# AleoNet/snarkVM

Hardware: NVIDIA H100
Metric: bls12_377_g1_msm_points_per_sec (higher is better)
Workload: dtype u32 limbs (Montgomery integer arithmetic, IMAD pipe)

## Files before the change

snarkvm_b200/csrc/msm.cu:

```cuda
#include "msm.cuh"

#include <atomic>
#include <condition_variable>
#include <memory>
#include <mutex>
#include <utility>
#include <vector>
#include <cstdio>
#include <cstdlib>
#include <cstring>
#include <cub/device/device_scan.cuh>

#define FF_CALL_MUL 1
#include "ec.cuh"
#include "cta_inverse.cuh"
#include "quad.cuh"
#define FIELD_TEST_ENTRY test_field_op_msm
#include "testops.cuh"

namespace b200 {

static std::atomic<uint64_t> g_launches{0};
uint64_t launch_count() { return g_launches.load(); }
void count_launch(int n) { g_launches.fetch_add((uint64_t)n); }
// ... 316 lines not shown
    acc.store(partial + (size_t)t * XYZZ_WORDS);
}

template <bool GATHER>
FF_DEV DensePoint load_level_input(const uint32_t* __restrict__ dense_bases, const uint32_t* __restrict__ sorted,
                                   const uint32_t* __restrict__ dense_in, uint32_t idx) {
    DensePoint d;
    if (GATHER) {
        uint32_t e = sorted[idx];
        d = load_dense(dense_bases + (size_t)(e & 0x7fffffffu) * BASE_WORDS);
        if ((e >> 31) && !d.inf) d.y = d.y.neg();
    } else {
        d = load_dense(dense_in + (size_t)idx * DENSE_WORDS);
    }
    return d;
}
template <bool GATHER>
FF_DEV const uint32_t* level_input_ptr(const uint32_t* __restrict__ dense_bases, const uint32_t* __restrict__ sorted,
                                       const uint32_t* __restrict__ dense_in, uint32_t idx) {
    if (GATHER) return dense_bases + (size_t)(sorted[idx] & 0x7fffffffu) * BASE_WORDS;
    return dense_in + (size_t)idx * DENSE_WORDS;
}
__global__ void k_densify_bases(const uint8_t* __restrict__ points, size_t stride, size_t n, uint32_t* __restrict__ out) {
    size_t i = (size_t)blockIdx.x * blockDim.x + threadIdx.x;
    if (i >= n) return;
    AffinePoint a = load_affine(points, stride, i);
    DensePoint d; d.x = a.x; d.y = a.y; d.inf = a.inf;
    store_dense(out + i * BASE_WORDS, d);
}
__global__ void __launch_bounds__(CTA_INV_THREADS) k_precompute_tables(const uint8_t* __restrict__ points, size_t stride, size_t n, int c, int nwin,
                                                            uint32_t* __restrict__ table) {
    __shared__ uint4 sh_inv[CTA_INV_SMEM_BYTES / 16];
    const size_t i = (size_t)blockIdx.x * blockDim.x + threadIdx.x;
    const bool live = i < n;
    AffinePoint a;
    a.x = Fq::zero(); a.y = Fq::zero(); a.inf = true;
    if (live) a = load_affine(points, stride, i);
    DensePoint d; d.x = a.x; d.y = a.y; d.inf = a.inf;
    if (live) store_dense(table + i * BASE_WORDS, d);
    XYZZ q = XYZZ::from_affine(a);
    for (int w = 1; w < nwin; w++) {
        for (int k = 0; k < c; k++) q.dbl();
        const bool inf = q.is_inf();
        Fq z = inf ? Fq::one() : q.ZZ * q.ZZZ;
        Fq iz = cta_shared_inverse_by(z, reinterpret_cast<uint32_t*>(sh_inv), w & 3);
        __syncthreads();
        if (inf) { d.x = Fq::zero(); d.y = Fq::zero(); d.inf = true; }
        else { d.x = q.X * (iz * q.ZZZ); d.y = q.Y * (iz * q.ZZ); d.inf = false; }
        if (live) store_dense(table + ((size_t)w * n + i) * BASE_WORDS, d);
    }
}

static constexpr int PAIR_THREADS = CTA_INV_THREADS;
enum PairKind { PAIR_COPY1 = 0, PAIR_COPY2 = 1, PAIR_INF = 2, PAIR_ADD = 3, PAIR_DBL = 4 };
FF_DEV int classify_pair(const DensePoint& P, const DensePoint& Q, bool has2, Fq& d) {
    if (!has2 || Q.inf) return PAIR_COPY1;
    if (P.inf) return PAIR_COPY2;
    if (P.x == Q.x) {
        if (P.y == Q.y && !P.y.is_zero()) { d = P.y.dbl(); return PAIR_DBL; }
        return PAIR_INF;
    }
    d = Q.x - P.x;
    return PAIR_ADD;
}

template <bool GATHER>
__global__ void __launch_bounds__(PAIR_THREADS, 4) k_pair_level(const uint32_t* __restrict__ dense_bases,
                                                        const uint32_t* __restrict__ sorted, const uint32_t* __restrict__ dense_in,
                                                        const uint32_t* __restrict__ off_in, const uint32_t* __restrict__ off_out,
                                                        uint32_t total_buckets, uint32_t T, uint32_t* __restrict__ prefix,
                                                        uint32_t* __restrict__ dense_out) {
    __shared__ uint4 sh_inv4[PAIR_THREADS * 3];
    uint32_t* sh_inv = reinterpret_cast<uint32_t*>(sh_inv4);
    const uint32_t total = off_out[total_buckets];
    const uint64_t o0_64 = (uint64_t)(blockIdx.x * blockDim.x + threadIdx.x) * T;
    const uint32_t o0 = o0_64 < total ? (uint32_t)o0_64 : total;
    const uint32_t o1 = (o0_64 + T < total) ? o0 + T : total;
    uint32_t lo = 0, hi = total_buckets;
    if (o0 < o1) while (hi - lo > 1) { uint32_t mid = (lo + hi) >> 1; if (off_out[mid] <= o0) lo = mid; else hi = mid; }
    uint32_t b = lo;

    Fq run = Fq::one();
    for (uint32_t o = o0; o < o1; o++) {
        while (o >= off_out[b + 1]) b++;
        const uint32_t i = o - off_out[b], base_in = off_in[b], cnt = off_in[b + 1] - base_in;
        const bool has2 = 2 * i + 1 < cnt;
        if (has2) {
            const uint32_t* pp = level_input_ptr<GATHER>(dense_bases, sorted, dense_in, base_in + 2 * i);
            const uint32_t* qp = level_input_ptr<GATHER>(dense_bases, sorted, dense_in, base_in + 2 * i + 1);
            Fq x1 = Fq::load_ldg(pp), x2 = Fq::load_ldg(qp);
            if (x1 == x2 || x1.is_zero() || x2.is_zero()) {
                DensePoint P = load_level_input<GATHER>(dense_bases, sorted, dense_in, base_in + 2 * i);
                DensePoint Q = load_level_input<GATHER>(dense_bases, sorted, dense_in, base_in + 2 * i + 1);
                Fq d;
                int kind = classify_pair(P, Q, true, d);
                if (kind >= PAIR_ADD) run = run * d;
            } else {
                run = run * (x2 - x1);
            }
        }
        run.store(prefix + (size_t)o * 12);
    }
    Fq inv = cta_shared_inverse(run, sh_inv);
    for (uint32_t o = o1; o-- > o0;) {
        while (o < off_out[b]) b--;
        const uint32_t i = o - off_out[b], base_in = off_in[b], cnt = off_in[b + 1] - base_in;
        const bool has2 = 2 * i + 1 < cnt;
        DensePoint P = load_level_input<GATHER>(dense_bases, sorted, dense_in, base_in + 2 * i);
        DensePoint Q = P;
        if (has2) Q = load_level_input<GATHER>(dense_bases, sorted, dense_in, base_in + 2 * i + 1);
        Fq d;
        int kind = classify_pair(P, Q, has2, d);
        DensePoint R;
        if (kind == PAIR_COPY1) R = P;
        else if (kind == PAIR_COPY2) R = Q;
        else if (kind == PAIR_INF) { R.inf = true; R.x = Fq::zero(); R.y = Fq::zero(); }
        else {
            Fq inv_d = (o == o0) ? inv : inv * Fq::load(prefix + (size_t)(o - 1) * 12);
            inv = inv * d;
            Fq lambda;
            if (kind == PAIR_ADD) lambda = (Q.y - P.y) * inv_d;
            else { Fq xx = P.x.sqr(); lambda = (xx.dbl() + xx) * inv_d; }
            Fq x3 = lambda.sqr() - P.x - Q.x;
            R.y = lambda * (P.x - x3) - P.y;
            R.x = x3;
            R.inf = false;
        }
        store_dense(dense_out + (size_t)o * DENSE_WORDS, R);
    }
}


FF_DEV uint32_t smem_addr_u32(const void* p) { return (uint32_t)__cvta_generic_to_shared(p); }
FF_DEV void cp_async16(uint32_t dst, const void* src) {
    asm volatile("cp.async.cg.shared.global [%0], [%1], 16;" ::"r"(dst), "l"(src) : "memory");
}
FF_DEV void cp_async_commit() { asm volatile("cp.async.commit_group;" ::: "memory"); }
FF_DEV void cp_async_wait_1() { asm volatile("cp.async.wait_group 1;" ::: "memory"); }
FF_DEV void cp_async_wait_0() { asm volatile("cp.async.wait_group 0;" ::: "memory"); }
FF_DEV void cp_async_wait_3() { asm volatile("cp.async.wait_group 3;" ::: "memory"); }

static constexpr int RING_CHUNKS = 12;
static constexpr int RING_STAGE_U4 = RING_CHUNKS * 32;
static constexpr int PAIR2_SMEM = PAIR_THREADS * 48 + 4 * 2 * RING_STAGE_U4 * 16;

FF_DEV Fq ring_fq(const uint4* slot) {
    Fq r;
#pragma unroll
    for (int i = 0; i < 3; i++) { uint4 t = slot[i * 32]; r.v[4 * i] = t.x; r.v[4 * i + 1] = t.y; r.v[4 * i + 2] = t.z; r.v[4 * i + 3] = t.w; }
    return r;
}

static constexpr uint32_t PAIR_NONE = 0xffffffffu;
template <bool GATHER>
__global__ void __launch_bounds__(256) k_pair_desc(const uint32_t* __restrict__ sorted, const uint32_t* __restrict__ off_in,
                                                   const uint32_t* __restrict__ off_out, uint32_t total_buckets, uint2* __restrict__ desc,
                                                   const uint32_t* __restrict__ in_base_ptr ) {
    const uint32_t o = blockIdx.x * blockDim.x + threadIdx.x;
    if (o >= __ldg(off_out + total_buckets)) return;
    uint32_t lo = 0, hi = total_buckets;
    while (hi - lo > 1) { uint32_t mid = (lo + hi) >> 1; if (__ldg(off_out + mid) <= o) lo = mid; else hi = mid; }
    const uint32_t i = o - __ldg(off_out + lo), base_in = __ldg(off_in + lo), cnt = __ldg(off_in + lo + 1) - base_in;
    const uint32_t idx = base_in + 2u * i;
    const bool has2 = 2u * i + 1u < cnt;
    uint2 d;
    if (GATHER) { d.x = __ldg(sorted + idx); d.y = has2 ? __ldg(sorted + idx + 1) : PAIR_NONE; }
    else { d.x = idx - (in_base_ptr ? __ldg(in_base_ptr) : 0u); d.y = has2 ? 0u : PAIR_NONE; }
    desc[o] = d;
}

struct PairDesc {
    uint32_t p, q;
    bool valid;
    FF_DEV bool has2() const { return valid && q != PAIR_NONE; }
};
FF_DEV PairDesc pair_load_desc(int64_t j, uint32_t nv, const uint2* __restrict__ dlane) {
    PairDesc d; d.p = 0; d.q = PAIR_NONE; d.valid = false;
    if (j < 0 || j >= (int64_t)nv) return d;
    const uint2 v = __ldg(dlane + 32 * j);
    d.p = v.x; d.q = v.y; d.valid = true;
    return d;
}
template <bool GATHER>
FF_DEV const uint32_t* pair_src(const PairDesc& d, int which, const uint32_t* __restrict__ records, uint32_t in_words) {
    if (GATHER) return records + (size_t)((which ? d.q : d.p) & 0x7fffffffu) * BASE_WORDS;
    return records + (size_t)(d.p + (uint32_t)which) * in_words;
}
template <bool GATHER, bool FULL>
FF_DEV void pair_issue(const PairDesc& d, uint4* ring, int st, int lane, const uint32_t* __restrict__ records, uint32_t in_words, int chunks) {
    if (d.valid) {
        const uint32_t dst = smem_addr_u32(ring + (size_t)st * (size_t)(chunks * 32) + lane);
        const uint32_t* p = pair_src<GATHER>(d, 0, records, in_words);
#pragma unroll
        for (int k = 0; k < (FULL ? 6 : 3); k++) cp_async16(dst + (uint32_t)k * 512u, p + 4 * k);
        if (d.q != PAIR_NONE) {
            const uint32_t* q = pair_src<GATHER>(d, 1, records, in_words);
#pragma unroll
            for (int k = 0; k < (FULL ? 6 : 3); k++) cp_async16(dst + (uint32_t)((FULL ? 6 : 3) + k) * 512u, q + 4 * k);
        }
    }
    cp_async_commit();
}
template <bool GATHER>
FF_DEV int pair_classify_global(const PairDesc& d, const uint32_t* __restrict__ records, uint32_t in_words, Fq& den) {
    DensePoint P = load_dense(pair_src<GATHER>(d, 0, records, in_words));
    DensePoint Q = load_dense(pair_src<GATHER>(d, 1, records, in_words));
    if (GATHER) { if ((d.p >> 31) && !P.inf) P.y = P.y.neg(); if ((d.q >> 31) && !Q.inf) Q.y = Q.y.neg(); }
    return classify_pair(P, Q, true, den);
}

template <bool GATHER, int MINB>
__global__ void __launch_bounds__(PAIR_THREADS, MINB) k_pair_level2(const uint32_t* __restrict__ records ,
                                                         uint32_t in_words, const uint2* __restrict__ desc, const uint32_t* __restrict__ total_ptr,
                                                         uint32_t T_bound, uint32_t* __restrict__ prefix, uint32_t* __restrict__ dense_out,
                                                         uint32_t* __restrict__ sm_slots) {
    (void)T_bound;
    extern __shared__ uint4 pair2_smem[];
    __shared__ uint32_t sh_slot;
    uint32_t* sh_inv = reinterpret_cast<uint32_t*>(pair2_smem);
    const int lane = threadIdx.x & 31, warp = threadIdx.x >> 5;
    uint4* ring = pair2_smem + PAIR_THREADS * 3 + (size_t)warp * 2 * RING_STAGE_U4;
    if (threadIdx.x == 0) {
        uint32_t smid;
        asm volatile("mov.u32 %0, %%smid;" : "=r"(smid));
        sh_slot = atomicAdd(sm_slots + (smid & 255u), 1u);
    }
    __syncthreads();
    const int inv_warp = (int)(sh_slot & 3u);
    const uint32_t total = __ldg(total_ptr);
    const uint64_t lanes = (uint64_t)gridDim.x * PAIR_THREADS;
    const uint32_t T = total > lanes ? (uint32_t)((total + lanes - 1) / lanes) : 1u;
    const uint64_t w0_64 = ((uint64_t)blockIdx.x * (PAIR_THREADS / 32) + (uint32_t)warp) * 32ull * T + (uint32_t)lane;
    uint32_t nv = 0;
    if (w0_64 < total) { const uint64_t left = (total - w0_64 + 31) / 32; nv = left < T ? (uint32_t)left : T; }
    const uint2* dlane = desc + w0_64;
    uint32_t* plane = prefix + w0_64 * 12;
    uint32_t* olane = dense_out + w0_64 * DENSE_WORDS;

    Fq run = Fq::one();
    {
        constexpr int PF = 3;
        PairDesc q0 = pair_load_desc(0, nv, dlane), q1 = pair_load_desc(1, nv, dlane), q2 = pair_load_desc(2, nv, dlane);
        pair_issue<GATHER, false>(q0, ring, 0, lane, records, in_words, 6);
        pair_issue<GATHER, false>(q1, ring, 1, lane, records, in_words, 6);
        pair_issue<GATHER, false>(q2, ring, 2, lane, records, in_words, 6);
        PairDesc ahead = pair_load_desc(PF, nv, dlane);
        for (uint32_t j = 0; j < T; j++) {
            pair_issue<GATHER, false>(ahead, ring, (int)((j + PF) & 3u), lane, records, in_words, 6);
            const PairDesc cur = q0;
            q0 = q1; q1 = q2; q2 = ahead;
            ahead = pair_load_desc((int64_t)j + PF + 1, nv, dlane);
            cp_async_wait_3();
            Fq d = Fq::one();
            if (cur.has2()) {
                const uint4* slot_p = ring + (size_t)(j & 3u) * (6 * 32) + lane;
                Fq x1 = ring_fq(slot_p), x2 = ring_fq(slot_p + 3 * 32);
                if (x1 == x2 || x1.is_zero() || x2.is_zero()) {
                    Fq den;
                    if (pair_classify_global<GATHER>(cur, records, in_words, den) >= PAIR_ADD) d = den;
                } else {
                    d = x2 - x1;
                }
            }
            run = run * d;
            if (cur.valid) run.store(plane + (size_t)j * (32 * 12));
        }
        cp_async_wait_0();
    }
    Fq inv = cta_shared_inverse_by(run, sh_inv, inv_warp);
    {
        PairDesc cur = pair_load_desc((int64_t)T - 1, nv, dlane);
        pair_issue<GATHER, true>(cur, ring, 0, lane, records, in_words, 12);
        PairDesc nxt = pair_load_desc((int64_t)T - 2, nv, dlane);
        for (uint32_t k = 0; k < T; k++) {
            const uint32_t j = T - 1 - k;
            pair_issue<GATHER, true>(nxt, ring, (int)((k + 1) & 1u), lane, records, in_words, 12);
            PairDesc nn = pair_load_desc((int64_t)j - 2, nv, dlane);
            Fq pf = Fq::one();
            if (cur.valid && j != 0) pf = Fq::load(plane + (size_t)(j - 1) * (32 * 12));
            cp_async_wait_1();
            const uint4* slot_p = ring + (size_t)(k & 1u) * RING_STAGE_U4 + lane;
            int kind = PAIR_COPY1;
            Fq d = Fq::one(), num = Fq::zero();
            const bool has2 = cur.has2();
            const bool negP = GATHER && (cur.p >> 31), negQ = GATHER && has2 && (cur.q >> 31);
            if (has2) {
                Fq x1 = ring_fq(slot_p), x2 = ring_fq(slot_p + 6 * 32);
                if (x1 == x2 || x1.is_zero() || x2.is_zero()) {
                    DensePoint P, Q;
                    P.x = x1; P.y = ring_fq(slot_p + 3 * 32); P.inf = P.x.is_zero() && P.y.is_zero();
                    Q.x = x2; Q.y = ring_fq(slot_p + 9 * 32); Q.inf = Q.x.is_zero() && Q.y.is_zero();
                    if (negP && !P.inf) P.y = P.y.neg();
                    if (negQ && !Q.inf) Q.y = Q.y.neg();
                    Fq den;
                    kind = classify_pair(P, Q, true, den);
                    if (kind >= PAIR_ADD) d = den;
                    if (kind == PAIR_ADD) num = Q.y - P.y;
                    else if (kind == PAIR_DBL) { Fq xx = P.x.sqr(); num = xx.dbl() + xx; }
                } else {
                    kind = PAIR_ADD;
                    d = x2 - x1;
                    Fq y1 = ring_fq(slot_p + 3 * 32), y2 = ring_fq(slot_p + 9 * 32);
                    if (negP == negQ) { num = y2 - y1; if (negP) num = num.neg(); }
                    else { num = y2 + y1; if (negQ) num = num.neg(); }
                }
            }
            Fq inv_next = inv * d;
            Fq inv_d = (j != 0) ? inv * pf : inv;
            inv = inv_next;
            Fq lambda = num * inv_d;
            Fq x3 = lambda.sqr();
            {
                Fq x1 = ring_fq(slot_p), x2 = has2 ? ring_fq(slot_p + 6 * 32) : x1;
                x3 = x3 - x1 - x2;
                Fq t = x1 - x3;
                Fq y3 = lambda * t;
                if (cur.valid) {
                    DensePoint R;
                    if (kind >= PAIR_ADD) {
                        Fq y1 = ring_fq(slot_p + 3 * 32);
                        R.x = x3; R.y = negP ? y3 + y1 : y3 - y1; R.inf = false;
// ... 735 lines not shown
        partial = a.take<uint32_t>(max_items * XYZZ_WORDS);
        partial2 = a.take<uint32_t>(((quad_fold || large_hot) ? max_items : (size_t)TBg + max_items / 32 + 2) * XYZZ_WORDS);
        hot_dev = a.take<uint32_t>(hot_max + 2);
        red_a = a.take<uint32_t>((size_t)gw * (2 * chunks_per_set > 2 * ((plan.nbuckets + 7u) / 8u) ? 2 * chunks_per_set : 2 * ((plan.nbuckets + 7u) / 8u)) * XYZZ_WORDS);
        red_b = a.take<uint32_t>((size_t)gw * (chunks_per_set / tree + 1 > 2 * ((plan.nbuckets + 63u) / 64u) + 2 ? chunks_per_set / tree + 1 : 2 * ((plan.nbuckets + 63u) / 64u) + 2) * XYZZ_WORDS);
        cub_tmp = a.take<uint8_t>(cub_bytes);
        if (!flat && !records) dense_bases = a.take<uint32_t>(total_bases * (size_t)BASE_WORDS);
        if (records) dense0 = a.take<uint32_t>(entries_g * (size_t)rec_words);
        if (levels > 0) {
            off_a = a.take<uint32_t>((size_t)TBg + 1);
            off_b = a.take<uint32_t>((size_t)TBg + 1);
            dense_a = a.take<uint32_t>(dense_cap_a * DENSE_WORDS);
            if (levels > 1) dense_b = records && dense_cap_b * DENSE_WORDS <= entries_g * (size_t)rec_words ? dense0 : a.take<uint32_t>(dense_cap_b * DENSE_WORDS);
            prefix = a.take<uint32_t>(dense_cap_a * 12);
            desc = a.take<uint2>(dense_cap_a);
            sm_slots = a.take<uint32_t>(256);
        }
    };
    layout(ar);
    const size_t scratch_bytes = ar.off;
    void* block = nullptr;
    DeviceScratch* ds = nullptr;
    if ((rc = scratch_acquire(&block, scratch_bytes, stream, &ds)) != 0) return rc;
    ar.base = (uint8_t*)block; ar.off = 0;
    layout(ar);

    CUDA_TRY(cudaMemsetAsync(hist, 0, (size_t)(TB + 1) * 4, stream));
    if (sm_slots) CUDA_TRY(cudaMemsetAsync(sm_slots, 0, 256 * 4, stream));
    if (quad_fold) CUDA_TRY(cudaMemsetAsync(hot_dev, 0, 4, stream));
    {
        {
            ProfScope sort_scope(PROF_MSM_SORT, stream);
            for (int pass = 0; pass < (records ? 1 : 2); pass++) {
                for (int i = 0; i < nsegs; i++) {
                    const MsmSegment& sg = segs[i];
                    if (sg.n == 0) continue;
                    const unsigned grid = (unsigned)((sg.n + 255) / 256);
                    const uint32_t slot_base = sg.job * sets_per_job * plan.nbuckets;
                    const uint32_t* sc = (const uint32_t*)sg.d_scalars;
                    const size_t fl = flat ? table_n : 0;
                    if (pass == 0) {
                        if (sg.mont) k_digits<false, true><<<grid, 256, 0, stream>>>(sc, sg.n, plan.c, plan.c_top, plan.nwin, plan.nbuckets, hist, nullptr, fl, slot_base, sg.base0, d_flags);
                        else k_digits<false, false><<<grid, 256, 0, stream>>>(sc, sg.n, plan.c, plan.c_top, plan.nwin, plan.nbuckets, hist, nullptr, fl, slot_base, sg.base0, d_flags);
                    } else {
                        if (sg.mont) k_digits<true, true><<<grid, 256, 0, stream>>>(sc, sg.n, plan.c, plan.c_top, plan.nwin, plan.nbuckets, cursors, sorted, fl, slot_base, sg.base0, d_flags);
                        else k_digits<true, false><<<grid, 256, 0, stream>>>(sc, sg.n, plan.c, plan.c_top, plan.nwin, plan.nbuckets, cursors, sorted, fl, slot_base, sg.base0, d_flags);
                    }
                    count_launch();
                }
                if (pass == 0) {
                    CUDA_TRY(cub::DeviceScan::ExclusiveSum(cub_tmp, cub_bytes, hist, bucket_start, (int)(TB + 1), stream));
                    CUDA_TRY(cudaMemcpyAsync(cursors, bucket_start, (size_t)(TB + 1) * 4, cudaMemcpyDeviceToDevice, stream));
                    count_launch(2);
                }
            }
        }
        const uint32_t* gather_src = flat ? table : dense_bases;
        if (!flat && !records) {
            ProfScope acc_scope(PROF_MSM_ACCUMULATE, stream);
            size_t at = 0;
            for (int i = 0; i < nbases; i++) {
                if (bases[i].n == 0) continue;
                k_densify_bases<<<(unsigned)((bases[i].n + 255) / 256), 256, 0, stream>>>((const uint8_t*)bases[i].d_points, bases[i].stride, bases[i].n,
                                                                                        dense_bases + at * BASE_WORDS);
                count_launch();
                at += bases[i].n;
            }
        }
        for (uint32_t u0 = 0; u0 < nwins; u0 += gu) {
            const uint32_t un = nwins - u0 < gu ? nwins - u0 : gu;
            const uint32_t w0 = set_of(u0), wn = set_of(u0 + un) - w0;
            const uint32_t tb = wn * plan.nbuckets;
            const uint32_t* bs = bucket_start + (size_t)w0 * plan.nbuckets;
            const SetOffsets so = set_offsets(plan, flat, w0);
            size_t entries = set_cap * (size_t)un;
            if (entries > max_entries) entries = max_entries;
            if (large_hot) CUDA_TRY(cudaMemsetAsync(hot_dev, 0, 4, stream));
            size_t items_bound = 1;
            size_t items_launched = 1;
            const uint32_t* final_partial = nullptr;
            const uint32_t* final_start = nullptr;
            if (levels == 0) {
                const uint32_t cap = (acc_g8 || acc_q8 || small_cap) ? item_cap : plan.cap;
                k_items_per_bucket<<<(tb + 256) / 256, 256, 0, stream>>>(hist + (size_t)w0 * plan.nbuckets, items, tb, cap, (quad_fold || large_hot) ? hot_dev : nullptr, (uint32_t)hot_max, hot_keep);
                CUDA_TRY(cub::DeviceScan::ExclusiveSum(cub_tmp, cub_bytes, items, item_start, (int)(tb + 1), stream));
                count_launch(2);
                const size_t group_items = (size_t)tb + entries / cap + 1;
                items_bound = set_cap / cap + 1;
                items_launched = group_items;
                ProfScope acc_scope(PROF_MSM_ACCUMULATE, stream);
                if (acc_q8) {
                    k_bucket_accumulate_q8<<<(unsigned)((group_items * 32 + 127) / 128), 128, 0, stream>>>(gather_src, sorted, bs, item_start, tb, cap, partial);
                    items_bound = 1;
                } else if (acc_g8)
                    k_bucket_accumulate_g8<<<(unsigned)((group_items * ACC_G + 127) / 128), 128, 0, stream>>>(gather_src, sorted, bs, item_start, tb, cap, partial);
                else
                    k_bucket_accumulate<<<(unsigned)((group_items + MSM_ACC_THREADS - 1) / MSM_ACC_THREADS), MSM_ACC_THREADS, 0, stream>>>(
                        gather_src, sorted, bs, item_start, tb, cap, partial);
                count_launch();
            } else {
                if (records) {
                    ProfScope sort_scope(PROF_MSM_SORT, stream);
                    for (int i = 0; i < nsegs; i++) {
                        const MsmSegment& sg = segs[i];
                        if (sg.n == 0) continue;
                        const int64_t first = (int64_t)sg.job * wins_per_job;
                        int w_lo, w_hi;
                        if (flat) {
                            if (first < (int64_t)u0 || first >= (int64_t)u0 + un) continue;
                            w_lo = 0; w_hi = plan.nwin;
                        } else {
                            const int64_t lo_w = (int64_t)u0 - first, hi_w = (int64_t)u0 + un - first;
                            w_lo = lo_w < 0 ? 0 : (int)lo_w; w_hi = hi_w > plan.nwin ? plan.nwin : (int)hi_w;
                            if (w_lo >= w_hi) continue;
                        }
                        const unsigned grid = (unsigned)((sg.n + 255) / 256);
                        const uint32_t slot_base = sg.job * sets_per_job * plan.nbuckets;
                        const uint32_t* sc = (const uint32_t*)sg.d_scalars;
                        const int ct = plan.c_top, nw = plan.nwin;
                        if (flat) {
                            if (sg.mont) k_scatter_records<true, true><<<grid, 256, 0, stream>>>(sc, sg.n, nullptr, 0, table, table_n, plan.c, ct, nw, plan.nbuckets, cursors, slot_base, w_lo, w_hi, bs, (uint4*)dense0, rec_words);
                            else k_scatter_records<false, true><<<grid, 256, 0, stream>>>(sc, sg.n, nullptr, 0, table, table_n, plan.c, ct, nw, plan.nbuckets, cursors, slot_base, w_lo, w_hi, bs, (uint4*)dense0, rec_words);
                        } else {
                            if (sg.mont) k_scatter_records<true, false><<<grid, 256, 0, stream>>>(sc, sg.n, seg_points[i], seg_stride[i], nullptr, 0, plan.c, ct, nw, plan.nbuckets, cursors, slot_base, w_lo, w_hi, bs, (uint4*)dense0, rec_words);
                            else k_scatter_records<false, false><<<grid, 256, 0, stream>>>(sc, sg.n, seg_points[i], seg_stride[i], nullptr, 0, plan.c, ct, nw, plan.nbuckets, cursors, slot_base, w_lo, w_hi, bs, (uint4*)dense0, rec_words);
                        }
                        count_launch();
                    }
                }
                ProfScope acc_scope(PROF_MSM_ACCUMULATE, stream);
                const uint32_t* off_in = bs;
                uint32_t* off_bufs[2] = {off_a, off_b};
                uint32_t* dense_bufs[2] = {dense_a, dense_b};
                const uint32_t* dense_in = records ? dense0 : nullptr;
                size_t bound = entries;
                for (int l = 0; l < levels; l++) {
                    uint32_t* off_out = off_bufs[l & 1];
                    uint32_t* dense_out = dense_bufs[l & 1];
                    k_halve_counts<<<(tb + 256) / 256, 256, 0, stream>>>(off_in, cnt_tmp, tb);
                    CUDA_TRY(cub::DeviceScan::ExclusiveSum(cub_tmp, cub_bytes, cnt_tmp, off_out, (int)(tb + 1), stream));
                    bound = bound / 2 + tb;
                    const size_t wave = (size_t)sm_count * (pair_v1 ? 4 : pair_minb) * 128;
                    size_t waves = (bound + 1024 * wave - 1) / (1024 * wave);
                    if (pair_waves) waves = pair_waves;
                    size_t T = (bound + waves * wave - 1) / (waves * wave);
                    const size_t nthreads = (bound + T - 1) / T;
                    const unsigned lgrid = (unsigned)((nthreads + 127) / 128);
                    if (pair_v1) {
                        if (l == 0 && !records)
                            k_pair_level<true><<<lgrid, 128, 0, stream>>>(gather_src, sorted, nullptr, off_in, off_out, tb, (uint32_t)T, prefix, dense_out);
                        else
                            k_pair_level<false><<<lgrid, 128, 0, stream>>>(nullptr, nullptr, dense_in, off_in, off_out, tb, (uint32_t)T, prefix, dense_out);
                    } else {
                        const unsigned dgrid = (unsigned)((bound + 255) / 256);
                        if (l == 0 && !records) {
                            k_pair_desc<true><<<dgrid, 256, 0, stream>>>(sorted, off_in, off_out, tb, desc, nullptr);
                            if (pair_minb == 3) k_pair_level2<true, 3><<<lgrid, 128, PAIR2_SMEM, stream>>>(gather_src, BASE_WORDS, desc, off_out + tb, (uint32_t)T, prefix, dense_out, sm_slots);
                            else k_pair_level2<true, 4><<<lgrid, 128, PAIR2_SMEM, stream>>>(gather_src, BASE_WORDS, desc, off_out + tb, (uint32_t)T, prefix, dense_out, sm_slots);
                        } else {
                            k_pair_desc<false><<<dgrid, 256, 0, stream>>>(nullptr, off_in, off_out, tb, desc, l == 0 ? bs : nullptr);
                            const uint32_t in_words = l == 0 ? rec_words : (uint32_t)DENSE_WORDS;
                            if (pair_minb == 3) k_pair_level2<false, 3><<<lgrid, 128, PAIR2_SMEM, stream>>>(dense_in, in_words, desc, off_out + tb, (uint32_t)T, prefix, dense_out, sm_slots);
                            else k_pair_level2<false, 4><<<lgrid, 128, PAIR2_SMEM, stream>>>(dense_in, in_words, desc, off_out + tb, (uint32_t)T, prefix, dense_out, sm_slots);
                        }
                        count_launch(1);
                    }
                    count_launch(3);
                    off_in = off_out;
                    dense_in = dense_out;
                }
                k_items_from_offsets<<<(tb + 256) / 256, 256, 0, stream>>>(off_in, items, tb, plan.cap, large_hot ? hot_dev : nullptr, (uint32_t)hot_max, hot_keep);
                CUDA_TRY(cub::DeviceScan::ExclusiveSum(cub_tmp, cub_bytes, items, item_start, (int)(tb + 1), stream));
                const size_t group_items = (size_t)tb + bound / plan.cap + 1;
                items_bound = ((set_cap >> levels) + 1) / plan.cap + 1;
                items_launched = group_items;
                k_bucket_accumulate_dense<<<(unsigned)((group_items + MSM_ACC_THREADS - 1) / MSM_ACC_THREADS), MSM_ACC_THREADS, 0, stream>>>(
                    dense_in, off_in, item_start, tb, plan.cap, partial);
                count_launch(3);
            }
            ProfScope red_scope(PROF_MSM_REDUCE, stream);
            int quad_rounds = 0;
            if (quad_fold) {
                size_t worst = acc_q8 ? 1 : items_bound;
                const uint32_t* p_in = partial; uint32_t* p_out = partial2;
                while (worst > 32) {
                    k_fold_hot_quad<<<(unsigned)sm_count * 8, 128, 0, stream>>>(p_in, item_start, hot_dev, (uint32_t)hot_max, (uint32_t)quad_rounds, 32u, p_out);
                    count_launch();
                    worst = (worst + 31) / 32;
                    quad_rounds++;
                    const uint32_t* t1 = p_in; p_in = p_out; p_out = (uint32_t*)t1;
                }
                final_partial = partial; final_start = item_start;
            } else if (large_hot) {
                size_t worst = items_bound;
                const uint32_t* p_in = partial; uint32_t* p_out = partial2;
                while (worst > 1) {
                    k_fold_hot_quad<<<(unsigned)sm_count * 8, 128, 0, stream>>>(p_in, item_start, hot_dev, (uint32_t)hot_max, (uint32_t)quad_rounds, 1u, p_out);
                    count_launch();
                    worst = (worst + 31) / 32;
                    quad_rounds++;
                    const uint32_t* t1 = p_in; p_in = p_out; p_out = (uint32_t*)t1;
                }
                final_partial = partial; final_start = item_start;
            } else {
                size_t worst = items_bound;
                size_t total_bound = items_launched;
                uint32_t* p_in = partial; uint32_t* p_out = partial2;
                uint32_t* st_in = item_start; uint32_t* st_out = items2;
                while (worst > 1) {
                    k_group_counts<<<(tb + 256) / 256, 256, 0, stream>>>(st_in, cnt_tmp, tb);
                    CUDA_TRY(cub::DeviceScan::ExclusiveSum(cub_tmp, cub_bytes, cnt_tmp, st_out, (int)(tb + 1), stream));
                    const size_t out_bound = (size_t)tb + total_bound / 32 + 1;
                    total_bound = out_bound;
                    k_partial_group_sum<<<(unsigned)((out_bound + 127) / 128), 128, 0, stream>>>(p_in, st_in, st_out, tb, p_out);
                    count_launch(3);
                    worst = (worst + 31) / 32;
                    uint32_t* t1 = p_in; p_in = p_out; p_out = t1;
                    uint32_t* t2 = st_in; st_in = st_out; st_out = t2;
                }
                final_partial = p_in; final_start = st_in;
            }
            uint32_t* group_sums = d_window_sums + (size_t)w0 * XYZZ_WORDS;
            if (warp_reduce && quad_path != 0) {
                const uint32_t qchunks = (plan.nbuckets + 7u) / 8u;
                k_bucket_reduce_quad<<<(wn * qchunks * 32u + 127u) / 128u, 128, 0, stream>>>(final_partial, quad_fold ? partial2 : final_partial, final_start,
                                                                                              quad_rounds, plan.nbuckets, qchunks, wn, red_a);
                const uint32_t* ent = red_a;
                uint32_t m = qchunks;
                int lgw = 3;
                if (m > 64u) {
                    const uint32_t groups = (m + 7u) / 8u;
                    k_combine_level_quad<<<(wn * groups * 32u + 127u) / 128u, 128, 0, stream>>>(ent, m, wn, lgw, red_b);
                    count_launch();
                    ent = red_b; m = groups; lgw += 3;
                }
                k_window_combine_quad<<<wn, 32u * ((m + 7u) / 8u), 0, stream>>>(ent, m, lgw, group_sums, so);
                count_launch(2);
                continue;
            }
            if (warp_reduce) {
                const uint32_t wchunks = (plan.nbuckets + 31u) / 32u;
                k_bucket_reduce_warp<<<(wn * wchunks * 32u + 127u) / 128u, 128, 0, stream>>>(final_partial, final_start, plan.nbuckets, wchunks, wn, red_a);
                k_window_combine_warp<<<wn, 32, 0, stream>>>(red_a, wchunks, group_sums, so);
                count_launch(2);
                continue;
            }
            const uint32_t nthreads = chunks_per_set * wn;
            if (quad_path != 0 && quad_tail_large) {
                k_bucket_reduce<true><<<(nthreads + 127) / 128, 128, 0, stream>>>(final_partial, final_start, plan.nbuckets, chunk, chunks_per_set, wn, red_a,
                                                                                    partial2, large_hot ? quad_rounds : 0);
                count_launch(1);
                const uint32_t* ent = red_a;
                uint32_t* other = red_b;
                uint32_t m = chunks_per_set;
                int lgw = 0;
                while ((1u << lgw) < chunk) lgw++;
                while (m > 64u) {
                    const uint32_t groups = (m + 7u) / 8u;
                    if ((size_t)wn * groups >= 2048)
                        k_combine_level_quadseq<<<(unsigned)(((size_t)wn * groups * 4 + 127) / 128), 128, 0, stream>>>(ent, m, wn, lgw, other);
                    else
                        k_combine_level_quad<<<(wn * groups * 32u + 127u) / 128u, 128, 0, stream>>>(ent, m, wn, lgw, other);
                    count_launch();
                    uint32_t* done = other; other = (uint32_t*)ent; ent = done;
                    m = groups; lgw += 3;
                }
                k_window_combine_quad<<<wn, 32u * ((m + 7u) / 8u), 0, stream>>>(ent, m, lgw, group_sums, so);
                count_launch();
                continue;
            }
            k_bucket_reduce<false><<<(nthreads + 127) / 128, 128, 0, stream>>>(final_partial, final_start, plan.nbuckets, chunk, chunks_per_set, wn, red_a,
                                                                                 nullptr, 0, so);
            count_launch(1);
            uint32_t per_row = chunks_per_set;
            const uint32_t* src = red_a;
            uint32_t* bufs[2] = {red_b, red_a};
            int which = 0;
            while (per_row > 1) {
                uint32_t out_per_row = (per_row + tree - 1) / tree;
                uint32_t* target = out_per_row == 1 ? group_sums : bufs[which];
                uint32_t nt = out_per_row * wn;
                k_group_sum<<<(nt + 127) / 128, 128, 0, stream>>>(src, per_row, tree, out_per_row, wn, target);
                count_launch();
                src = target; which ^= 1; per_row = out_per_row;
            }
            if (chunks_per_set == 1)
                CUDA_TRY(cudaMemcpyAsync(group_sums, red_a, (size_t)wn * XYZZ_WORDS * 4, cudaMemcpyDeviceToDevice, stream));
        }
        CUDA_TRY(cudaGetLastError());
    }
done:
    scratch_release(block, scratch_bytes, stream, ds);
    return rc;
}

size_t msm_scan_bytes(size_t count) {
    size_t bytes = 0;
    cub::DeviceScan::ExclusiveSum(nullptr, bytes, (uint32_t*)nullptr, (uint32_t*)nullptr, (int)count);
    return bytes < 16 ? 16 : bytes;
}
int msm_exclusive_scan(void* tmp, size_t tmp_bytes, const uint32_t* in, uint32_t* out, size_t count, cudaStream_t stream) {
    count_launch(2);
    return (int)cub::DeviceScan::ExclusiveSum(tmp, tmp_bytes, in, out, (int)count, stream);
}
int msm_sort_indices(const MsmPlan& plan, const void* d_scalars, size_t n, int mont, uint32_t* hist, uint32_t* bucket_start, uint32_t* cursors,
                     uint32_t* sorted, void* cub_tmp, size_t cub_bytes, uint32_t* d_flags, cudaStream_t stream) {
    if (plan.nsets != plan.nwin || plan.c_top != plan.c) return (int)cudaErrorInvalidValue;
// ... 316 lines not shown
```

Baseline: 169.0 million.

## Replace per-thread binary search in pair descriptor kernel with warp-cooperative bucket walk

The pair descriptor kernel now assigns each warp a run of 8x32 consecutive outputs. It does one binary search per warp, then resolves bucket membership for the lanes with ballots, reduce-or and shuffles over a window of 32 bucket offsets, advancing the bucket cursor step by step. A per-lane binary search remains as a fallback when the window does not cover all outputs. This removes most of the per-thread log(buckets) dependent global loads, at the cost of more complex warp logic and fewer threads launched.

```diff
diff --git a/snarkvm_b200/csrc/msm.cu b/snarkvm_b200/csrc/msm.cu
--- a/snarkvm_b200/csrc/msm.cu
+++ b/snarkvm_b200/csrc/msm.cu
@@ -492,21 +492,52 @@
 }
 
 static constexpr uint32_t PAIR_NONE = 0xffffffffu;
+static constexpr uint32_t PAIR_DESC_STEPS = 8;
 template <bool GATHER>
 __global__ void __launch_bounds__(256) k_pair_desc(const uint32_t* __restrict__ sorted, const uint32_t* __restrict__ off_in,
                                                    const uint32_t* __restrict__ off_out, uint32_t total_buckets, uint2* __restrict__ desc,
                                                    const uint32_t* __restrict__ in_base_ptr ) {
-    const uint32_t o = blockIdx.x * blockDim.x + threadIdx.x;
-    if (o >= __ldg(off_out + total_buckets)) return;
-    uint32_t lo = 0, hi = total_buckets;
-    while (hi - lo > 1) { uint32_t mid = (lo + hi) >> 1; if (__ldg(off_out + mid) <= o) lo = mid; else hi = mid; }
-    const uint32_t i = o - __ldg(off_out + lo), base_in = __ldg(off_in + lo), cnt = __ldg(off_in + lo + 1) - base_in;
-    const uint32_t idx = base_in + 2u * i;
-    const bool has2 = 2u * i + 1u < cnt;
-    uint2 d;
-    if (GATHER) { d.x = __ldg(sorted + idx); d.y = has2 ? __ldg(sorted + idx + 1) : PAIR_NONE; }
-    else { d.x = idx - (in_base_ptr ? __ldg(in_base_ptr) : 0u); d.y = has2 ? 0u : PAIR_NONE; }
-    desc[o] = d;
+    const uint32_t lane = threadIdx.x & 31u;
+    const uint32_t total = __ldg(off_out + total_buckets);
+    const uint64_t w0_64 = ((uint64_t)blockIdx.x * (blockDim.x / 32) + (threadIdx.x >> 5)) * (32ull * PAIR_DESC_STEPS);
+    if (w0_64 >= total) return;
+    const uint32_t w0 = (uint32_t)w0_64;
+    const uint32_t in_base = in_base_ptr ? __ldg(in_base_ptr) : 0u;
+    uint32_t c = 0, hi = total_buckets;
+    while (hi - c > 1) { const uint32_t mid = (c + hi) >> 1; if (__ldg(off_out + mid) <= w0) c = mid; else hi = mid; }
+    for (uint32_t s = 0; s < PAIR_DESC_STEPS; s++) {
+        const uint32_t o0 = w0 + 32u * s;
+        if (o0 >= total) break;
+        const uint32_t kw = min(c + lane, total_buckets);
+        const uint32_t oo = __ldg(off_out + kw), oi = __ldg(off_in + kw);
+        const uint32_t last = min(o0 + 31u, total - 1u);
+        const uint32_t o = min(o0 + lane, last);
+        const uint32_t a = oo - o0;
+        const bool before = lane >= 1 && oo <= o0, inside = lane >= 1 && oo > o0 && a <= 31u;
+        const uint32_t marks = __reduce_or_sync(0xffffffffu, inside ? 1u << a : 0u);
+        const bool fits = __shfl_sync(0xffffffffu, oo, 31) > last && __popc(__ballot_sync(0xffffffffu, inside)) == __popc(marks);
+        uint32_t b, ob, ib, ib1;
+        if (fits) {
+            const uint32_t r = __popc(__ballot_sync(0xffffffffu, before)) + __popc(marks & ((2u << (o - o0)) - 1u));
+            b = c + r;
+            ob = __shfl_sync(0xffffffffu, oo, r); ib = __shfl_sync(0xffffffffu, oi, r); ib1 = __shfl_sync(0xffffffffu, oi, r + 1u);
+        } else {
+            uint32_t lo = c, h = total_buckets;
+            while (h - lo > 1) { const uint32_t mid = (lo + h) >> 1; if (__ldg(off_out + mid) <= o) lo = mid; else h = mid; }
+            b = lo;
+            ob = __ldg(off_out + b); ib = __ldg(off_in + b); ib1 = __ldg(off_in + b + 1);
+        }
+        const uint32_t idx = ib + 2u * (o - ob);
+        const bool has2 = idx + 1u < ib1;
+        if (o0 + lane < total) {
+            uint2 d;
+            if (GATHER) { d.x = __ldg(sorted + idx); d.y = has2 ? __ldg(sorted + idx + 1) : PAIR_NONE; }
+            else { d.x = idx - in_base; d.y = has2 ? 0u : PAIR_NONE; }
+            desc[o0 + lane] = d;
+        }
+        const uint32_t n = __popc(__ballot_sync(0xffffffffu, oo <= o0 + 32u));
+        c = fits ? c + n - 1u : __shfl_sync(0xffffffffu, b, 31);
+    }
 }
 
 struct PairDesc {
@@ -1548,7 +1579,7 @@
                         else
                             k_pair_level<false><<<lgrid, 128, 0, stream>>>(nullptr, nullptr, dense_in, off_in, off_out, tb, (uint32_t)T, prefix, dense_out);
                     } else {
-                        const unsigned dgrid = (unsigned)((bound + 255) / 256);
+                        const unsigned dgrid = (unsigned)((bound + 8 * 32 * PAIR_DESC_STEPS - 1) / (8 * 32 * PAIR_DESC_STEPS));
                         if (l == 0 && !records) {
                             k_pair_desc<true><<<dgrid, 256, 0, stream>>>(sorted, off_in, off_out, tb, desc, nullptr);
                             if (pair_minb == 3) k_pair_level2<true, 3><<<lgrid, 128, PAIR2_SMEM, stream>>>(gather_src, BASE_WORDS, desc, off_out + tb, (uint32_t)T, prefix, dense_out, sm_slots);
```

Result: faster. 173.7 million, median of 6 (+2.8%).
